# starreeze/drin

Measured on AMD Instinct MI355X. Metric: mention x candidate pairs scored/sec, higher is better.
Workload: dtype bf16x3; 1 GPU; wikimel-shaped scoring forward: 100-cand (+1 answer slot), D=768, R=2048, L=128, P=49, T=64 token-level entity text; parallelism=dp1 (mentions sharded, no collective)

## Files before the change

drin_amd/_lib.py:

```python
from __future__ import annotations

import ctypes as C
import os
from typing import Optional

_HERE = os.path.dirname(os.path.abspath(__file__))
LIB_PATH = os.environ.get("DRIN_LIB_PATH") or os.path.join(_HERE, "libdrin_hip.so")
MAX_LAYERS = 8
ABI_VERSION = 12

OK, E_SHAPE, E_NULL, E_ALIGN, E_WORKSPACE, E_HIP, E_UNSUPPORTED, E_INDEX = 0, -1, -2, -3, -4, -5, -6, -7
PREC_F32, PREC_BF16X3, PREC_BF16X3_ALL, PREC_BF16X3_IF16 = 0, 1, 3, 5
FEAT_F32, FEAT_BF16 = 0, 1
CACHE_F32, CACHE_MIXED_F16 = 0, 1
CACHE_FORMATS = {"f32": CACHE_F32, "mixed_f16": CACHE_MIXED_F16}
ACTIVATIONS = {"gelu": 1, "sigmoid": 2, "relu": 3, "tanh": 4, "silu": 5}

fp = C.POINTER(C.c_float)
ip = C.POINTER(C.c_int64)


class DrinConfigC(C.Structure):
    _fields_ = [
        ("batch", C.c_int32), ("num_candidates", C.c_int32), ("embed_dim", C.c_int32), ("image_dim", C.c_int32),
# ... 113 lines not shown
EXPORTS = {
    "drin_version": (C.c_int, []),
    "drin_last_error": (C.c_char_p, []),
    "drin_build_info": (C.c_char_p, []),
    "drin_default_config": (C.c_int, [C.POINTER(DrinConfigC)]),
    "drin_host_selftest": (C.c_int, []),
    "drin_workspace_bytes": (C.c_size_t, [C.POINTER(DrinConfigC), C.c_int]),
    "drin_edges_fwd": (C.c_int, [C.POINTER(DrinConfigC), C.POINTER(DrinBatchC), C.c_void_p, C.c_void_p, C.c_void_p]),
    "drin_pool_fwd": (C.c_int, [C.POINTER(DrinConfigC), C.POINTER(DrinBatchC), C.c_void_p, C.c_void_p, C.c_void_p, C.c_void_p]),
    "drin_linear_fwd": (C.c_int, [C.c_void_p, C.c_void_p, C.c_void_p, C.c_void_p, C.c_int64, C.c_int32, C.c_int32, C.c_int32, C.c_void_p]),
    "drin_linear_bwd": (C.c_int, [C.c_void_p, C.c_void_p, C.c_void_p, C.c_void_p, C.c_void_p, C.c_void_p, C.c_int64, C.c_int32,
                                  C.c_int32, C.c_int32, C.c_void_p, C.c_size_t, C.c_void_p]),
    "drin_forward": (C.c_int, [C.POINTER(DrinConfigC), C.POINTER(DrinBatchC), C.POINTER(DrinParamsC), C.c_void_p,
                               C.c_size_t, C.c_void_p, C.c_int, C.POINTER(DrinTraceC), C.c_void_p]),
    "drin_forward_staged": (C.c_int, [C.POINTER(DrinConfigC), C.POINTER(DrinBatchC), C.POINTER(DrinParamsC), C.c_void_p,
                                      C.c_size_t, C.c_void_p, C.c_int, C.POINTER(DrinTraceC), C.c_void_p, C.c_void_p]),
    "drin_backward": (C.c_int, [C.POINTER(DrinConfigC), C.POINTER(DrinBatchC), C.POINTER(DrinParamsC), C.c_void_p,
                                C.c_size_t, C.c_void_p, C.POINTER(DrinParamGradsC), C.c_void_p]),
    "drin_backward_staged": (C.c_int, [C.POINTER(DrinConfigC), C.POINTER(DrinBatchC), C.POINTER(DrinParamsC), C.c_void_p,
                                       C.c_size_t, C.c_void_p, C.POINTER(DrinParamGradsC), C.c_void_p, C.c_void_p]),
    "drin_backward_ex": (C.c_int, [C.POINTER(DrinConfigC), C.POINTER(DrinBatchC), C.POINTER(DrinParamsC), C.c_void_p,
                                   C.c_size_t, C.c_void_p, C.POINTER(DrinParamGradsC), C.POINTER(DrinInputGradsC), C.c_void_p,
                                   C.c_void_p]),
    "drin_input_grad_scratch_bytes": (C.c_size_t, [C.POINTER(DrinConfigC)]),
    "drin_pool_bwd": (C.c_int, [C.POINTER(DrinConfigC), C.c_void_p, C.c_void_p, C.c_void_p, C.c_void_p, C.c_void_p]),
    "drin_fused_supported": (C.c_int, [C.POINTER(DrinConfigC)]),
    "drin_indexed_supported": (C.c_int, [C.POINTER(DrinConfigC)]),
    "drin_prepared_bytes": (C.c_size_t, [C.POINTER(DrinConfigC)]),
    "drin_fused_workspace_bytes": (C.c_size_t, [C.POINTER(DrinConfigC)]),
    "drin_workgroups_per_mention": (C.c_int32, [C.POINTER(DrinConfigC), C.c_int32]),
    "drin_index_status": (C.c_int, [C.c_void_p, C.c_void_p]),
    "drin_image_contraction_passes": (C.c_int32, [C.POINTER(DrinConfigC), C.c_int32]),
    "drin_image_contraction_side_tiles": (C.c_int32, [C.POINTER(DrinConfigC), C.c_int32]),
    "drin_prepare": (C.c_int, [C.POINTER(DrinConfigC), C.POINTER(DrinParamsC), C.c_void_p, C.c_size_t, C.c_void_p]),
    "drin_forward_prepared": (C.c_int, [C.POINTER(DrinConfigC), C.POINTER(DrinBatchC), C.POINTER(DrinParamsC), C.c_void_p,
                                        C.c_void_p, C.c_size_t, C.c_void_p, C.c_void_p]),
    "drin_entity_cache_bytes": (C.c_size_t, [C.POINTER(DrinConfigC)]),
    "drin_entity_cache_build_workspace_bytes": (C.c_size_t, [C.POINTER(DrinConfigC)]),
    "drin_cached_workspace_bytes": (C.c_size_t, [C.POINTER(DrinConfigC)]),
    "drin_build_entity_cache": (C.c_int, [C.POINTER(DrinConfigC), C.POINTER(DrinBatchC), C.POINTER(DrinParamsC), C.c_void_p,
                                          C.c_void_p, C.c_size_t, C.c_void_p, C.c_size_t, C.c_void_p]),
    "drin_forward_cached": (C.c_int, [C.POINTER(DrinConfigC), C.POINTER(DrinBatchC), C.POINTER(DrinParamsC), C.c_void_p,
                                      C.c_void_p, C.c_void_p, C.c_size_t, C.c_void_p, C.c_void_p]),
    "drin_split_planes": (C.c_int, [C.c_void_p, C.c_void_p, C.c_void_p, C.c_int64, C.c_void_p]),
    "drin_linear_planes_fwd": (C.c_int, [C.c_void_p, C.c_void_p, C.c_void_p, C.c_void_p, C.c_void_p, C.c_void_p,
                                         C.c_int64, C.c_int32, C.c_int32, C.c_void_p]),
    "drin_gemm_probe": (C.c_int, [C.POINTER(DrinGemmProbeArgsC), C.c_void_p]),
    "drin_loss_workspace_bytes": (C.c_size_t, [C.c_int32]),
    "drin_triplet_topk": (C.c_int, [C.c_void_p, C.c_void_p, C.c_int32, C.c_int32, C.c_float, C.POINTER(C.c_int32), C.c_int32,
                                    C.c_void_p, C.c_void_p, C.c_void_p, C.c_void_p, C.c_size_t, C.c_void_p]),
    "drin_adam_step": (C.c_int, [C.c_void_p, C.c_void_p, C.c_void_p, C.c_void_p, C.c_int64, C.c_float, C.c_float, C.c_float,
                                 C.c_float, C.c_float, C.c_float, C.c_void_p]),
    "drin_melhi_workspace_bytes": (C.c_size_t, [C.POINTER(DrinMelhiConfigC), C.c_int]),
    "drin_melhi_forward": (C.c_int, [C.POINTER(DrinMelhiConfigC), C.POINTER(DrinMelhiBatchC), C.POINTER(DrinMelhiParamsC), C.c_void_p,
                                     C.c_void_p, C.c_void_p, C.c_size_t, C.c_void_p, C.c_void_p]),
    "drin_melhi_backward": (C.c_int, [C.POINTER(DrinMelhiConfigC), C.POINTER(DrinMelhiBatchC), C.POINTER(DrinMelhiParamsC),
                                      C.c_void_p, C.c_void_p, C.c_void_p, C.c_size_t, C.c_void_p, C.POINTER(DrinMelhiParamGradsC),
                                      C.c_void_p]),
    "drin_ghmfc_workspace_bytes": (C.c_size_t, [C.POINTER(DrinGhmfcConfigC)]),
    "drin_ghmfc_forward": (C.c_int, [C.POINTER(DrinGhmfcConfigC), C.POINTER(DrinGhmfcBatchC), C.POINTER(DrinGhmfcParamsC), C.c_void_p,
                                     C.c_size_t, C.c_void_p, C.c_void_p, C.c_void_p]),
    "drin_attention": (C.c_int, [C.c_void_p, C.c_int64, C.c_void_p, C.c_int64, C.c_void_p, C.c_int64, C.c_void_p, C.c_void_p, C.c_int64,
                                 C.c_int32, C.c_int32, C.c_int32, C.c_int32, C.c_int32, C.c_void_p]),
    "drin_attention_train_fwd": (C.c_int, [C.c_void_p, C.c_int64, C.c_void_p, C.c_int64, C.c_void_p, C.c_int64, C.c_void_p, C.c_void_p,
                                           C.c_int64, C.c_void_p, C.c_int32, C.c_int32, C.c_int32, C.c_int32, C.c_int32, C.c_void_p]),
    "drin_attention_bwd": (C.c_int, [C.c_void_p, C.c_int64, C.c_void_p, C.c_int64, C.c_void_p, C.c_int64, C.c_void_p, C.c_void_p,
                                     C.c_int64, C.c_void_p, C.c_void_p, C.c_int64, C.c_void_p, C.c_int64, C.c_void_p, C.c_int64,
                                     C.c_void_p, C.c_int64, C.c_void_p, C.c_int32, C.c_int32, C.c_int32, C.c_int32, C.c_int32,
                                     C.c_void_p]),
# ... 54 lines not shown
```

drin_amd/build.py:

```python
from __future__ import annotations

import os
import subprocess
import sys
from concurrent.futures import ThreadPoolExecutor

HERE = os.path.dirname(os.path.abspath(__file__))
CSRC = os.path.join(HERE, "csrc")
INCLUDE = os.path.join(os.path.dirname(HERE), "include")
LIB = os.path.join(HERE, "libdrin_hip.so")
ARCH = "gfx950"
SOURCES = ["api.hip", "stream_kernels.hip", "gemm_f32.hip", "gemm_bf16x3.hip", "gemm_x3_planes.hip", "gemm_tn_bf16x3.hip", "gcn_kernels.hip", "backward_kernels.hip", "fused_kernels.hip", "fused_forward.hip", "vector_kernels.hip", "loss_kernels.hip", "entity_cache.hip", "optim_kernels.hip", "input_grad_kernels.hip", "melhi_kernels.hip", "ghmfc_kernels.hip"]


def _hipcc() -> str:
    for c in (os.environ.get("HIPCC"), "/opt/rocm/bin/hipcc", "hipcc"):
        if c and (os.path.isabs(c) and os.path.exists(c) or not os.path.isabs(c)):
            return c
    raise RuntimeError("hipcc not found")


def _newest_header() -> float:
    hs = [os.path.join(CSRC, f) for f in os.listdir(CSRC) if f.endswith(".h")]
    hs += [os.path.join(INCLUDE, f) for f in os.listdir(INCLUDE) if f.endswith(".h")]
    return max(os.path.getmtime(h) for h in hs)


ASAN_LIB = os.path.join(HERE, "libdrin_hip_asan.so")
SAN_FLAGS = ["-fsanitize=address,undefined", "-fno-gpu-sanitize", "-fno-omit-frame-pointer", "-fno-sanitize-recover=undefined", "-g"]


def asan_runtime() -> str:
    out = subprocess.run([_hipcc(), "-print-file-name=libclang_rt.asan-x86_64.so"], capture_output=True, text=True).stdout.strip()
    if not os.path.isabs(out) or not os.path.exists(out):
        import glob
        hits = sorted(glob.glob("/opt/rocm/lib/llvm/lib/clang/*/lib/linux/libclang_rt.asan-x86_64.so"))
        if not hits:
            raise RuntimeError("clang's libclang_rt.asan-x86_64.so not found")
        out = hits[-1]
    return out


def build(force: bool = False, debug: bool = False, verbose: bool = True, asan_host: bool = False, variant: str = "") -> str:
    obj_dir = os.path.join(CSRC, "build_asan" if asan_host else ("build_" + variant if variant else "build"))
    os.makedirs(obj_dir, exist_ok=True)
# ... 49 lines not shown
```

drin_amd/csrc/fused.h:

```cpp
#pragma once
#include <hip/hip_runtime.h>
#include <stddef.h>
#include <stdint.h>
#include <string.h>

#include "../../include/drin_hip.h"
#include "layout.h"

namespace drin {

struct Prepared {
  size_t wcat1, bcat1, ecat, etmp, k_t, k_i, c_txt, c_img, cb_t, cb_i, total;
  size_t p_ctxt, p_cimg, p_wh2;
  size_t p_wmt, p_wmi, p_wcat1, p_ecat, p_wet, p_wei, p_wh1;
  size_t p_cimg_f16;
  size_t cimg_f16_scale;
  void build(const drin_config& c) {
    const size_t D = c.embed_dim, R = c.image_dim;
    size_t off = 0;
    auto take = [&off](size_t n) {
      const size_t o = off;
      off += (n + 63) & ~(size_t)63;
      return o;
    };
// ... 89 lines not shown
  const float* gamma;
  const float* beta;
  const float* e1m;
  const float* mt2;
  float* scores;
  int B, N, D4, chunks;
  int act_v;
  float ln_eps, cos_eps;
};

template <class Args>
Args shaped_args(const drin_config& c) {
  Args a;
  memset(&a, 0, sizeof(a));
  a.B = c.batch, a.N = c.num_candidates, a.D4 = c.embed_dim / 4;
  return a;
}
template <class Args>
void set_vertex_fields(Args& a, const drin_config& c) {
  a.ln_eps = c.layer_norm_eps, a.act_v = vertex_act(&c);
}
template <class Args>
void set_edge_fields(Args& a, const drin_config& c) {
  a.R4 = c.image_dim / 4;
  a.Km = c.mention_objects;
  a.dynamic = c.dynamic_edges != 0;
  a.act_e = edge_act(&c);
  for (int k = 0; k < 4; ++k) a.mask[k] = c.edge_enabled[k];
  a.cos_eps = c.cosine_eps, a.miei_eps = c.miei_eps, a.clip = c.clip_scale;
}

size_t entity_stream_lds_bytes(const StreamArgs& a);
int launch_entity_stream(const StreamArgs& a, hipStream_t st);
int launch_reduce_stream_partials(const float* part, float* s_text, float* s_img, float* sig, int B, int D, int R,
                                  int chunks, hipStream_t st);
int launch_mention_input1(const float* T, const float* T2, const float* sig, const float* b_et, const float* b_ei,
                          const float* v0, float* out, int B, int D, int N, hipStream_t st);
int launch_pair_layer1(const PairArgs& a, hipStream_t st);
int launch_mention_input2(const float* part, const float* mt1, float* out, int B, int D, int N, int chunks,
                          hipStream_t st);
int launch_pair_final(const FinalArgs& a, hipStream_t st);

struct GemmScratch {
  float* p = nullptr;
  size_t floats = 0;
};
int run_folded_head(const drin_config* cfg, const drin_batch* b, const drin_params* params, const float* prepared, const Prepared& P,
                    bool weight_planes, float* span_mean, float* mimg, float* vm0, float* hmfu, GemmScratch mention_sk, hipStream_t st);
int run_folded_mention_finish(const drin_config* cfg, const drin_params* params, const float* prepared, const Prepared& P,
                              bool weight_planes, float* vm1, float* hm2, GemmScratch mention_sk, hipStream_t st);
int run_folded_tail(const drin_config* cfg, const drin_params* params, const float* prepared, const Prepared& P, int chunks,
                    const float* s2_part, const float* vm1, float* agg2, float* mt2, const float* hm2, const float* e1m, float* h2,
                    const float* et1, const void* et1_hi, bool weight_planes, GemmScratch mention_sk, GemmScratch pair_sk,
                    float* scores, hipStream_t st);
}
```

drin_amd/csrc/fused_forward.hip:

```cpp
#include <string.h>

#include "fused.h"
#include "internal.h"
#include "layout.h"

namespace drin {

constexpr int kMixedMinCandidates = 64;

struct FusedLayout {
  size_t span_mean, mimg, vm0, hmfu, q, e0m, e1m, xt, s_part, s_text, s_img, sig, tm, tm2, agg1, vm1, hm2, h_text, h_image,
      et1, s2_part, agg2, mt2, p_xt, p_xi, p_et1, xi_scale, splitk, splitk_floats, pair_splitk, pair_splitk_floats, total;
  int chunks;
  void build(const drin_config& c) {
    const size_t B = c.batch, N = c.num_candidates, D = c.embed_dim, R = c.image_dim, M = B * N;
    chunks = (int)(B >= 2048 ? (N + 127) / 128 : B >= 1024 ? (N + 47) / 48 : (N + 15) / 16);
    size_t off = 0;
    auto take = [&off](size_t n) {
      const size_t o = off;
      off += (n + 63) & ~(size_t)63;
      return o;
    };
    span_mean = take(B * D);
    mimg = take(B * R);
// ... 63 lines not shown
#ifdef DRIN_SIDE_PROBE
static int g_probe_wgs = kSideWgs, g_probe_permille = kSidePermille;
extern "C" __attribute__((visibility("default"))) void drin_probe_side_plan(int wgs, int permille) { g_probe_wgs = wgs, g_probe_permille = permille; }
#endif
struct SidePlan {
  int64_t S = 0;
  int G = 0;
};
static SidePlan image_side_plan(const drin_config* c, bool indexed, bool capturing) {
  SidePlan plan;
  int wgs = kSideWgs, permille = kSidePermille;
#ifdef DRIN_SIDE_PROBE
  wgs = g_probe_wgs, permille = g_probe_permille;
#endif
  const bool split = c->precision == DRIN_PREC_BF16X3 || c->precision == DRIN_PREC_BF16X3_ALL || c->precision == DRIN_PREC_BF16X3_IF16;
  if (capturing || indexed || !split || if16_gate(c, indexed) || wgs <= 0 || permille <= 0) return plan;
  const int D = c->embed_dim, R = c->image_dim;
  if ((D % 32) || (R % 32) || c->batch <= 0) return plan;
  const int64_t M = (int64_t)c->batch * c->num_candidates;
  const int64_t nx = cdiv(D, 256), row_tiles = cdiv(M, 256), tiles = row_tiles * nx;
  if (tiles < 192 || tiles < kSideMinTiles || tiles > ((int64_t)1 << 28)) return plan;
  FusedLayout L;
  L.build(*c);
  const int64_t whole_rows = gemm_p4_whole_tiles(tiles, R, L.splitk_floats > 0, L.splitk_floats) / nx;
  int64_t S = (row_tiles * permille + 500) / 1000;
  S = S < whole_rows ? S : whole_rows;
  S = S < row_tiles - 1 ? S : row_tiles - 1;
  if (S <= 0) return plan;
  plan.S = S;
  plan.G = (int)(wgs < S * nx ? wgs : S * nx);
  return plan;
}

struct SideJoin {
  SideLane* lane = nullptr;
  hipStream_t st = nullptr;
  int join() {
    if (!lane) return DRIN_OK;
    const hipError_t e = hipStreamWaitEvent(st, lane->join, 0);
    lane = nullptr;
    return e == hipSuccess ? DRIN_OK : hip_fail(e, "hipStreamWaitEvent(side stream)");
  }
  ~SideJoin() { (void)join(); }
};

int fused_supported(const drin_config* c) {
  if (c->num_layers != 2) {
    set_error("fused path: built for num_layers == 2 (got %d); use drin_forward", c->num_layers);
    return DRIN_E_UNSUPPORTED;
  }
  if (c->vector_edges) {
    set_error("fused path: vector edge features (model.py:112-116) run on the layer-by-layer path; use drin_forward");
    return DRIN_E_UNSUPPORTED;
  }
  if (c->mention_object_inner > 1 || c->entity_object_inner > 1 || c->entity_image_inner > 1) {
    set_error("fused path: inner feature dims > 1 need the pooled path of drin_forward");
    return DRIN_E_UNSUPPORTED;
  }
  const bool tiny = c->embed_dim <= 256 && c->image_dim <= 256;
  const bool full = c->embed_dim <= 768 && c->image_dim <= 2048;
  if (!tiny && !full) {
    set_error("fused path: D=%d R=%d outside the built instantiations", c->embed_dim, c->image_dim);
    return DRIN_E_UNSUPPORTED;
  }
  return DRIN_OK;
}
// ... 138 lines not shown
                    const float* et1, const void* et1_hi, bool weight_planes, GemmScratch sk, GemmScratch pair_sk, float* scores,
                    hipStream_t st) {
  const int B = cfg->batch, N = cfg->num_candidates, D = cfg->embed_dim, prec = folded_precision(cfg);
  const int64_t M = (int64_t)B * N;
  const drin_layer_params& L2 = params->layer[1];
  DRIN_TRY(launch_mention_input2(s2_part, vm1, agg2, B, D, N, chunks, st));
  DRIN_TRY(launch_gemm_nt(agg2, D, L2.w_h, D, L2.b_h, mt2, D, B, D, D, false, prec, st, sk.p, sk.floats,
                          weight_planes ? pb + P.p_wh2 : nullptr));
  DRIN_TRY(launch_layernorm_gelu(mt2, L2.ln_weight, L2.ln_bias, mt2, nullptr, nullptr, B, D, cfg->layer_norm_eps, st, vertex_act(cfg)));
  if (et1_hi) {
    const __bf16* e1 = static_cast<const __bf16*>(et1_hi);
    const __bf16* w2 = reinterpret_cast<const __bf16*>(pb + P.p_wh2);
    DRIN_TRY(launch_gemm_x3_planes(e1, e1 + (size_t)M * D, D, w2, w2 + (size_t)D * D, D, nullptr, h2, D, M, D, D, st, pair_sk.p,
                                   pair_sk.floats));
  } else {
    DRIN_TRY(launch_gemm_nt(et1, D, L2.w_h, D, nullptr, h2, D, M, D, D, false, prec, st));
  }
  FinalArgs fa = shaped_args<FinalArgs>(*cfg);
  set_vertex_fields(fa, *cfg);
  fa.h2 = h2;
  fa.hm2 = hm2;
  fa.b_h2 = L2.b_h;
  fa.gamma = L2.ln_weight;
  fa.beta = L2.ln_bias;
  fa.e1m = e1m;
  fa.mt2 = mt2;
  fa.scores = scores;
  fa.chunks = chunks;
  fa.cos_eps = cfg->cosine_eps;
  return launch_pair_final(fa, st);
}

static int forward_prepared_on_stream(const drin_config* cfg, const drin_batch* b, const drin_params* params, const void* prepared,
                                      void* workspace, float* scores, hipStream_t st) {
  FusedLayout L;
  L.build(*cfg);
  Prepared P;
  P.build(*cfg);
  float* ws = (float*)workspace;
  const float* pb = (const float*)prepared;
  const int B = cfg->batch, N = cfg->num_candidates, D = cfg->embed_dim, R = cfg->image_dim;
  const int64_t M = (int64_t)B * N;
  if (B == 0) return DRIN_OK;
  const int prec = folded_precision(cfg);
  const bool dyn = cfg->dynamic_edges != 0;
  const bool tokens = cfg->entity_tokens > 0;
  const bool planes = (prec == DRIN_PREC_BF16X3 || prec == DRIN_PREC_BF16X3_ALL) && (D % 32 == 0) && (R % 32 == 0);
  const bool indexed = b->entity_index != nullptr;
  const bool xi_planes = planes && indexed;
  const bool if16 = if16_gate(cfg, indexed) && gemm_f16_planes_fits(ws + L.p_xi, R, pb + P.p_cimg_f16, R, ws + L.h_image, D, M, D, R);
  hipStreamCaptureStatus capture = hipStreamCaptureStatusNone;
  if (hipStreamIsCapturing(st, &capture) != hipSuccess) {
    (void)hipGetLastError();
    capture = hipStreamCaptureStatusActive;
  }
  SidePlan side = image_side_plan(cfg, indexed, capture != hipStreamCaptureStatusNone);
  if (!aligned16(b->entity_image) || !aligned16(ws + L.h_image) || !b->entity_image) side = SidePlan();
  if (b->entity_text_cls) {
    set_error("drin_forward_prepared: entity_text_cls (text pooled ahead of time) is a form of the training entry points");
    return DRIN_E_UNSUPPORTED;
  }
  if (indexed && cfg->num_entities <= 0) {
    set_error("drin_forward_prepared: entity_index given but cfg.num_entities = %d", cfg->num_entities);
    return DRIN_E_SHAPE;
  }
  if (indexed && !planes) {
    set_error("drin_forward_prepared: entity_index needs the split-bf16 precision (the stream kernel gathers the "
// ... 55 lines not shown
  sa.index_status = b->index_status;
  sa.miet = b->miet_similarity;
  sa.mtei = b->mtei_similarity;
  sa.span_mean = ws + L.span_mean;
  sa.mobj = b->mention_object;
  sa.mscore = b->mention_object_score;
  sa.fu = hmfu + D;
  sa.ldfu = 2 * D;
  sa.q = ws + L.q;
  sa.ldq = D + R;
  sa.k_t = pb + P.k_t;
  sa.k_i = pb + P.k_i;
  sa.xt_out = planes ? nullptr : ws + L.xt;
  if (planes) {
    sa.xt_hi = xt_hi;
    sa.xt_lo = xt_exact ? nullptr : xt_hi + MD;
    if (xi_planes) {
      sa.xi_hi = xi_hi;
      sa.xi_lo = bf16_feat ? nullptr : xi_hi + MR;
    }
  }
  sa.xi_scale = if16 ? ws + L.xi_scale : nullptr;
  sa.xi_f16 = if16 ? static_cast<void*>(xi_hi) : nullptr;
  sa.e0m = ws + L.e0m;
  sa.e1m = ws + L.e1m;
  sa.s_part = ws + L.s_part;
  sa.T = cfg->entity_tokens;
  sa.Ke = cfg->entity_objects;
  sa.chunks = L.chunks;
  sa.bf16_features = bf16_feat ? 1 : 0;
  sa.s_text = ws + L.s_text;
  sa.s_img = ws + L.s_img;
  sa.sig = ws + L.sig;
  DRIN_TRY(launch_entity_stream(sa, st));
  if (L.chunks > 1)
    DRIN_TRY(launch_reduce_stream_partials(ws + L.s_part, ws + L.s_text, ws + L.s_img, ws + L.sig, B, D, R, L.chunks, st));
  DRIN_TRY(launch_gemm_nt_pair({ws + L.s_text, params->w_entity_text, nullptr, ws + L.tm, D, D, D, 2 * (int64_t)B, D, D, wp(P.p_wet)},
                               {ws + L.s_img, params->w_entity_image, nullptr, ws + L.tm2, R, R, D, 2 * (int64_t)B, D, R,
                                wp(P.p_wei)},
                               prec, st, msk.p, msk.floats));
  DRIN_TRY(launch_mention_input1(ws + L.tm, ws + L.tm2, ws + L.sig, params->b_entity_text, params->b_entity_image, vm0, ws + L.agg1, B, D, N, st));
  float* vm1 = ws + L.vm1;
  DRIN_TRY(launch_gemm_nt(ws + L.agg1, D, L1.w_h, D, L1.b_h, vm1, D, 2 * (int64_t)B, D, D, false, prec, st, msk.p, msk.floats, wp(P.p_wh1)));
  DRIN_TRY(run_folded_mention_finish(cfg, params, pb, P, planes, vm1, ws + L.hm2, msk, st));
  if (planes) {
    const __bf16* ct = reinterpret_cast<const __bf16*>(pb + P.p_ctxt);
    const __bf16* ci = reinterpret_cast<const __bf16*>(pb + P.p_cimg);
    DRIN_TRY(launch_gemm_x3_planes(xt_hi, xt_exact ? nullptr : xt_hi + MD, D, ct, ct + (size_t)D * D, D, nullptr, ws + L.h_text, D, M, D,
                                   D, st, psk.p, psk.floats));
    if (if16)
      DRIN_TRY(launch_gemm_f16_planes(xi_hi, R, pb + P.p_cimg_f16, R, ws + L.xi_scale, pb + P.cimg_f16_scale, ws + L.h_image, D, M, D, R,
                                      st, psk.p, psk.floats));
    else if (xi_planes)
      DRIN_TRY(launch_gemm_x3_planes(xi_hi, bf16_feat ? nullptr : xi_hi + MR, R, ci, ci + (size_t)D * R, R, nullptr, ws + L.h_image, D, M,
                                     D, R, st, psk.p, psk.floats));
    else if (side.S > 0) {
      DRIN_TRY(side_join.join());
      DRIN_TRY(image_rows_product(st, RowTiles{side.S, -1, 0}));
    } else if (bf16_feat)
      DRIN_TRY(launch_gemm_x3_planes(b->entity_image, nullptr, R, ci, ci + (size_t)D * R, R, nullptr, ws + L.h_image, D, M, D, R, st, psk.p,
                                     psk.floats));
    else
      DRIN_TRY(launch_gemm_nt_bf16x3(b->entity_image, R, pb + P.c_img, R, nullptr, ws + L.h_image, D, M, D, R, st, ci, ci + (size_t)D * R,
                                     false, psk.p, psk.floats));
  } else {
    const float* x_t = tokens ? ws + L.xt : b->entity_text;
    DRIN_TRY(launch_gemm_nt(x_t, D, pb + P.c_txt, D, nullptr, ws + L.h_text, D, M, D, D, false, prec, st));
    DRIN_TRY(launch_gemm_nt(b->entity_image, R, pb + P.c_img, R, nullptr, ws + L.h_image, D, M, D, R, false, prec, st));
  }
// ... 8 lines not shown
  pa.gamma = L1.ln_weight;
  pa.beta = L1.ln_bias;
  pa.e0m = ws + L.e0m;
  pa.e1m = ws + L.e1m;
  pa.et1 = planes ? nullptr : ws + L.et1;
  if (planes) {
    pa.et1_hi = e1_hi;
    pa.et1_lo = e1_hi + MD;
  }
  pa.s2_part = ws + L.s2_part;
  pa.chunks = L.chunks;
  DRIN_TRY(launch_pair_layer1(pa, st));
  return run_folded_tail(cfg, params, pb, P, L.chunks, ws + L.s2_part, vm1, ws + L.agg2, ws + L.mt2, ws + L.hm2, ws + L.e1m, ws + L.h_text,
                         planes ? nullptr : ws + L.et1, planes ? e1_hi : nullptr, planes, msk, psk, scores, st);
}

}

extern "C" {

int32_t drin_workgroups_per_mention(const drin_config* cfg, int32_t cached) {
  if (validate_config(cfg) != DRIN_OK || fused_supported(cfg) != DRIN_OK) return 0;
  if (cached) return cached_chunks_per_mention(*cfg);
  FusedLayout L;
  L.build(*cfg);
  return L.chunks;
}

int32_t drin_image_contraction_side_tiles(const drin_config* cfg, int32_t indexed) {
  if (validate_config(cfg) != DRIN_OK || fused_supported(cfg) != DRIN_OK) return 0;
  return (int32_t)image_side_plan(cfg, indexed != 0, false).S;
}

int32_t drin_image_contraction_passes(const drin_config* cfg, int32_t indexed) {
  if (validate_config(cfg) != DRIN_OK || fused_supported(cfg) != DRIN_OK) return 0;
  if (cfg->precision == DRIN_PREC_F32) return 0;
  if (if16_gate(cfg, indexed != 0)) return 1;
  return cfg->feature_dtype == DRIN_FEAT_BF16 ? 2 : 3;
}

int drin_index_status(int32_t* index_status, void* stream) {
  if (!index_status) {
    set_error("drin_index_status: NULL argument");
    return DRIN_E_NULL;
  }
  DRIN_BIND_DEVICE(stream, index_status, "drin_index_status");
  int32_t w[4] = {0, 0, 0, 0};
  hipError_t e = hipMemcpyAsync(w, index_status, sizeof(w), hipMemcpyDeviceToHost, (hipStream_t)stream);
  if (e == hipSuccess) e = hipStreamSynchronize((hipStream_t)stream);
  if (e != hipSuccess) return hip_fail(e, "drin_index_status");
  if (w[0] == 0) return DRIN_OK;
  e = hipMemsetAsync(index_status, 0, sizeof(w), (hipStream_t)stream);
  if (e != hipSuccess) return hip_fail(e, "drin_index_status(reset)");
  const long long value = (long long)(((uint64_t)(uint32_t)w[3] << 32) | (uint32_t)w[2]);
  set_error("entity_index out of range: candidate row %lld at pair %d (b * N + n) is outside the entity tables - the row was clamped "
            "and a WRONG entity scored; drin/data.py:87-93 raises IndexError here", value, (int)w[1]);
  return DRIN_E_INDEX;
}

size_t drin_fused_workspace_bytes(const drin_config* cfg) {
  if (validate_config(cfg) != DRIN_OK || fused_supported(cfg) != DRIN_OK) return 0;
  FusedLayout L;
  L.build(*cfg);
  return L.total * sizeof(float);
}

int drin_forward_prepared(const drin_config* cfg, const drin_batch* b, const drin_params* params, const void* prepared,
                          void* workspace, size_t workspace_bytes, float* scores, void* stream) {
  DRIN_BIND_DEVICE(stream, workspace, "drin_forward_prepared");
  RoctxRange range("drin_forward_prepared");
  DRIN_TRY(validate_config(cfg));
  DRIN_TRY(fused_supported(cfg));
  if (!b || !params || !prepared || !workspace || !scores) {
    set_error("drin_forward_prepared: NULL argument");
    return DRIN_E_NULL;
  }
  FusedLayout L;
  L.build(*cfg);
  if (workspace_bytes < L.total * sizeof(float) || !aligned16(workspace)) {
    set_error("drin_forward_prepared: workspace has %zu bytes (needs %zu) or is not 16-byte aligned", workspace_bytes,
              L.total * sizeof(float));
    return DRIN_E_WORKSPACE;
  }
  return forward_prepared_on_stream(cfg, b, params, prepared, workspace, scores, (hipStream_t)stream);
}

}
```

include/drin_hip.h:

```cpp
#ifndef DRIN_HIP_H_
#define DRIN_HIP_H_

#include <stddef.h>
#include <stdint.h>

#ifdef __cplusplus
extern "C" {
#endif

#define DRIN_ABI_VERSION 12
#define DRIN_API __attribute__((visibility("default")))

typedef enum {
  DRIN_OK = 0,
  DRIN_E_SHAPE = -1,
  DRIN_E_NULL = -2,
  DRIN_E_ALIGN = -3,
  DRIN_E_WORKSPACE = -4,
  DRIN_E_HIP = -5,
  DRIN_E_UNSUPPORTED = -6,
  DRIN_E_INDEX = -7
} drin_status;

typedef enum {
// ... 141 lines not shown
                 void* workspace, size_t workspace_bytes, float* scores, int keep_for_backward,
                 const drin_trace* trace, void* params_ready_event, void* stream);

DRIN_API int drin_backward(const drin_config* cfg, const drin_batch* batch, const drin_params* params,
                  void* workspace, size_t workspace_bytes, const float* grad_scores,
                  const drin_param_grads* grads, void* stream);

DRIN_API int drin_backward_staged(const drin_config* cfg, const drin_batch* batch, const drin_params* params,
                  void* workspace, size_t workspace_bytes, const float* grad_scores,
                  const drin_param_grads* grads, void* layers_ready_event, void* stream);

DRIN_API int drin_backward_ex(const drin_config* cfg, const drin_batch* batch, const drin_params* params,
                              void* workspace, size_t workspace_bytes, const float* grad_scores,
                              const drin_param_grads* grads, const drin_input_grads* input_grads,
                              void* layers_ready_event, void* stream);
DRIN_API size_t drin_input_grad_scratch_bytes(const drin_config* cfg);

DRIN_API int drin_pool_bwd(const drin_config* cfg, const int64_t* entity_text_mask, const float* grad_pooled,
                           const float* grad_cls, void* grad_entity_text, void* stream);

DRIN_API int drin_fused_supported(const drin_config* cfg);
DRIN_API size_t drin_prepared_bytes(const drin_config* cfg);
DRIN_API size_t drin_fused_workspace_bytes(const drin_config* cfg);
DRIN_API int drin_prepare(const drin_config* cfg, const drin_params* params, void* prepared, size_t prepared_bytes,
                          void* stream);
DRIN_API int drin_forward_prepared(const drin_config* cfg, const drin_batch* batch, const drin_params* params,
                                   const void* prepared, void* workspace, size_t workspace_bytes, float* scores,
                                   void* stream);
DRIN_API int32_t drin_workgroups_per_mention(const drin_config* cfg, int32_t cached);

DRIN_API int32_t drin_image_contraction_passes(const drin_config* cfg, int32_t indexed);

DRIN_API int32_t drin_image_contraction_side_tiles(const drin_config* cfg, int32_t indexed);

DRIN_API int drin_index_status(int32_t* index_status, void* stream);

DRIN_API size_t drin_entity_cache_bytes(const drin_config* cfg);
DRIN_API size_t drin_entity_cache_build_workspace_bytes(const drin_config* cfg);
DRIN_API size_t drin_cached_workspace_bytes(const drin_config* cfg);
DRIN_API int drin_build_entity_cache(const drin_config* cfg, const drin_batch* tables, const drin_params* params,
                                     const void* prepared, void* cache, size_t cache_bytes, void* workspace,
                                     size_t workspace_bytes, void* stream);
DRIN_API int drin_forward_cached(const drin_config* cfg, const drin_batch* batch, const drin_params* params,
                                 const void* prepared, const void* cache, void* workspace, size_t workspace_bytes,
                                 float* scores, void* stream);

DRIN_API int drin_split_planes(const float* x, void* hi, void* lo, int64_t n, void* stream);
DRIN_API int drin_linear_planes_fwd(const void* x_hi, const void* x_lo, const void* w_hi, const void* w_lo,
                                    const float* bias, float* y, int64_t rows, int32_t n_out, int32_t k,
                                    void* stream);

enum drin_gemm_probe_op {
  DRIN_PROBE_GEMM_NT = 1,
  DRIN_PROBE_GEMM_NT_BF16X3 = 2,
  DRIN_PROBE_GEMM_NT_BF16X3_P4 = 3,
  DRIN_PROBE_GEMM_X3_PLANES = 4,
  DRIN_PROBE_GEMM_F16_PLANES = 5,
  DRIN_PROBE_TO_F16_SCALED = 6
};
enum drin_gemm_family {
  DRIN_GEMM_FAMILY_NONE = 0,
  DRIN_GEMM_FAMILY_BF16X3 = 1,
  DRIN_GEMM_FAMILY_BF16X3_P4 = 2,
  DRIN_GEMM_FAMILY_PLANES = 3,
  DRIN_GEMM_FAMILY_PLANES_P4 = 4,
  DRIN_GEMM_FAMILY_F32 = 5,
// ... 184 lines not shown
```

Measured before the change: 28.06 million pairs/s.

## Add workgroup-per-mention walk kernel for the entity stream pass

Adds a new kernel that assigns one 256-thread workgroup per mention. The four waves split the token rows of each candidate, and the next candidate's rows are prefetched while the current one is reduced. When the config fits (fp32 features, D=768, R=2048, one entity object row, more than 16 candidates, a single chunk), it replaces the pair-per-wave entity stream kernel and the partial-reduction launch. The intent is better memory-level parallelism across token rows and fewer launches, at the cost of only B workgroups in the grid and heavy LDS use that may limit occupancy. A probe entry point is added to force either path.

```diff
diff --git a/drin_amd/_lib.py b/drin_amd/_lib.py
--- a/drin_amd/_lib.py
+++ b/drin_amd/_lib.py
@@ -169,9 +169,12 @@
     "drin_index_status": (C.c_int, [C.c_void_p, C.c_void_p]),
     "drin_image_contraction_passes": (C.c_int32, [C.POINTER(DrinConfigC), C.c_int32]),
     "drin_image_contraction_side_tiles": (C.c_int32, [C.POINTER(DrinConfigC), C.c_int32]),
+    "drin_stream_walk": (C.c_int32, [C.POINTER(DrinConfigC), C.c_int32]),
     "drin_prepare": (C.c_int, [C.POINTER(DrinConfigC), C.POINTER(DrinParamsC), C.c_void_p, C.c_size_t, C.c_void_p]),
     "drin_forward_prepared": (C.c_int, [C.POINTER(DrinConfigC), C.POINTER(DrinBatchC), C.POINTER(DrinParamsC), C.c_void_p,
                                         C.c_void_p, C.c_size_t, C.c_void_p, C.c_void_p]),
+    "drin_forward_prepared_probe": (C.c_int, [C.POINTER(DrinConfigC), C.POINTER(DrinBatchC), C.POINTER(DrinParamsC), C.c_void_p,
+                                              C.c_void_p, C.c_size_t, C.c_void_p, C.c_int32, C.c_void_p]),
     "drin_entity_cache_bytes": (C.c_size_t, [C.POINTER(DrinConfigC)]),
     "drin_entity_cache_build_workspace_bytes": (C.c_size_t, [C.POINTER(DrinConfigC)]),
     "drin_cached_workspace_bytes": (C.c_size_t, [C.POINTER(DrinConfigC)]),
diff --git a/drin_amd/build.py b/drin_amd/build.py
--- a/drin_amd/build.py
+++ b/drin_amd/build.py
@@ -10,7 +10,7 @@
 INCLUDE = os.path.join(os.path.dirname(HERE), "include")
 LIB = os.path.join(HERE, "libdrin_hip.so")
 ARCH = "gfx950"
-SOURCES = ["api.hip", "stream_kernels.hip", "gemm_f32.hip", "gemm_bf16x3.hip", "gemm_x3_planes.hip", "gemm_tn_bf16x3.hip", "gcn_kernels.hip", "backward_kernels.hip", "fused_kernels.hip", "fused_forward.hip", "vector_kernels.hip", "loss_kernels.hip", "entity_cache.hip", "optim_kernels.hip", "input_grad_kernels.hip", "melhi_kernels.hip", "ghmfc_kernels.hip"]
+SOURCES = ["api.hip", "stream_kernels.hip", "gemm_f32.hip", "gemm_bf16x3.hip", "gemm_x3_planes.hip", "gemm_tn_bf16x3.hip", "gcn_kernels.hip", "backward_kernels.hip", "fused_kernels.hip", "stream_walk.hip", "fused_forward.hip", "vector_kernels.hip", "loss_kernels.hip", "entity_cache.hip", "optim_kernels.hip", "input_grad_kernels.hip", "melhi_kernels.hip", "ghmfc_kernels.hip"]
 
 
 def _hipcc() -> str:
diff --git a/drin_amd/csrc/fused.h b/drin_amd/csrc/fused.h
--- a/drin_amd/csrc/fused.h
+++ b/drin_amd/csrc/fused.h
@@ -145,6 +145,9 @@
 
 size_t entity_stream_lds_bytes(const StreamArgs& a);
 int launch_entity_stream(const StreamArgs& a, hipStream_t st);
+bool mention_walk_built(const StreamArgs& a);
+size_t mention_walk_lds_bytes(const StreamArgs& a);
+int launch_mention_walk(const StreamArgs& a, hipStream_t st);
 int launch_reduce_stream_partials(const float* part, float* s_text, float* s_img, float* sig, int B, int D, int R,
                                   int chunks, hipStream_t st);
 int launch_mention_input1(const float* T, const float* T2, const float* sig, const float* b_et, const float* b_ei,
diff --git a/drin_amd/csrc/fused_forward.hip b/drin_amd/csrc/fused_forward.hip
--- a/drin_amd/csrc/fused_forward.hip
+++ b/drin_amd/csrc/fused_forward.hip
@@ -119,6 +119,17 @@
   return plan;
 }
 
+static bool stream_walk_built(const drin_config* c, bool indexed) {
+  return !indexed && c->feature_dtype == DRIN_FEAT_F32 && c->entity_tokens > 0 && c->embed_dim == 768 && c->image_dim == 2048 &&
+         c->entity_objects == 1 && c->mention_objects <= 11 && c->precision != DRIN_PREC_BF16X3_IF16;
+}
+static int stream_walk_route(const drin_config* c, bool indexed) {
+  if (!stream_walk_built(c, indexed) || c->num_candidates <= 16) return 0;
+  FusedLayout L;
+  L.build(*c);
+  return L.chunks == 1 ? 1 : 0;
+}
+
 struct SideJoin {
   SideLane* lane = nullptr;
   hipStream_t st = nullptr;
@@ -323,7 +334,7 @@
 }
 
 static int forward_prepared_on_stream(const drin_config* cfg, const drin_batch* b, const drin_params* params, const void* prepared,
-                                      void* workspace, float* scores, hipStream_t st) {
+                                      void* workspace, float* scores, hipStream_t st, int forced_walk = -1) {
   FusedLayout L;
   L.build(*cfg);
   Prepared P;
@@ -445,9 +456,15 @@
   sa.s_text = ws + L.s_text;
   sa.s_img = ws + L.s_img;
   sa.sig = ws + L.sig;
-  DRIN_TRY(launch_entity_stream(sa, st));
-  if (L.chunks > 1)
-    DRIN_TRY(launch_reduce_stream_partials(ws + L.s_part, ws + L.s_text, ws + L.s_img, ws + L.sig, B, D, R, L.chunks, st));
+  const int walk = forced_walk < 0 ? stream_walk_route(cfg, indexed) : forced_walk;
+  if (walk == 1) {
+    sa.chunks = 1;
+    DRIN_TRY(launch_mention_walk(sa, st));
+  } else {
+    DRIN_TRY(launch_entity_stream(sa, st));
+    if (L.chunks > 1)
+      DRIN_TRY(launch_reduce_stream_partials(ws + L.s_part, ws + L.s_text, ws + L.s_img, ws + L.sig, B, D, R, L.chunks, st));
+  }
   DRIN_TRY(launch_gemm_nt_pair({ws + L.s_text, params->w_entity_text, nullptr, ws + L.tm, D, D, D, 2 * (int64_t)B, D, D, wp(P.p_wet)},
                                {ws + L.s_img, params->w_entity_image, nullptr, ws + L.tm2, R, R, D, 2 * (int64_t)B, D, R,
                                 wp(P.p_wei)},
@@ -522,6 +539,11 @@
   return (int32_t)image_side_plan(cfg, indexed != 0, false).S;
 }
 
+int32_t drin_stream_walk(const drin_config* cfg, int32_t indexed) {
+  if (validate_config(cfg) != DRIN_OK || fused_supported(cfg) != DRIN_OK) return 0;
+  return stream_walk_route(cfg, indexed != 0);
+}
+
 int32_t drin_image_contraction_passes(const drin_config* cfg, int32_t indexed) {
   if (validate_config(cfg) != DRIN_OK || fused_supported(cfg) != DRIN_OK) return 0;
   if (cfg->precision == DRIN_PREC_F32) return 0;
@@ -555,24 +577,50 @@
   return L.total * sizeof(float);
 }
 
+static int forward_prepared_checked(const char* who, const drin_config* cfg, const drin_batch* b, const drin_params* params,
+                                    const void* prepared, void* workspace, size_t workspace_bytes, float* scores, int forced_walk,
+                                    void* stream) {
+  DRIN_TRY(validate_config(cfg));
+  DRIN_TRY(fused_supported(cfg));
+  if (!b || !params || !prepared || !workspace || !scores) {
+    set_error("%s: NULL argument", who);
+    return DRIN_E_NULL;
+  }
+  if (forced_walk > 1 || forced_walk < -1) {
+    set_error("%s: stream_walk %d (0: a pair per wave, 1: a pair per workgroup)", who, forced_walk);
+    return DRIN_E_SHAPE;
+  }
+  if (forced_walk == 1 && !stream_walk_built(cfg, b->entity_index != nullptr)) {
+    set_error("%s: the workgroup walk of the entity stream pass is built for fp32-stored gathered rows with token features at D = 768, "
+              "R = 2048, one entity object row and no fp16 image hand-over", who);
+    return DRIN_E_UNSUPPORTED;
+  }
+  FusedLayout L;
+  L.build(*cfg);
+  if (workspace_bytes < L.total * sizeof(float) || !aligned16(workspace)) {
+    set_error("%s: workspace has %zu bytes (needs %zu) or is not 16-byte aligned", who, workspace_bytes, L.total * sizeof(float));
+    return DRIN_E_WORKSPACE;
+  }
+  return forward_prepared_on_stream(cfg, b, params, prepared, workspace, scores, (hipStream_t)stream, forced_walk);
+}
+
 int drin_forward_prepared(const drin_config* cfg, const drin_batch* b, const drin_params* params, const void* prepared,
                           void* workspace, size_t workspace_bytes, float* scores, void* stream) {
   DRIN_BIND_DEVICE(stream, workspace, "drin_forward_prepared");
   RoctxRange range("drin_forward_prepared");
-  DRIN_TRY(validate_config(cfg));
-  DRIN_TRY(fused_supported(cfg));
-  if (!b || !params || !prepared || !workspace || !scores) {
-    set_error("drin_forward_prepared: NULL argument");
-    return DRIN_E_NULL;
-  }
-  FusedLayout L;
-  L.build(*cfg);
-  if (workspace_bytes < L.total * sizeof(float) || !aligned16(workspace)) {
-    set_error("drin_forward_prepared: workspace has %zu bytes (needs %zu) or is not 16-byte aligned", workspace_bytes,
-              L.total * sizeof(float));
-    return DRIN_E_WORKSPACE;
-  }
-  return forward_prepared_on_stream(cfg, b, params, prepared, workspace, scores, (hipStream_t)stream);
-}
-
-}
+  return forward_prepared_checked("drin_forward_prepared", cfg, b, params, prepared, workspace, workspace_bytes, scores, -1, stream);
+}
+
+int drin_forward_prepared_probe(const drin_config* cfg, const drin_batch* b, const drin_params* params, const void* prepared,
+                                void* workspace, size_t workspace_bytes, float* scores, int32_t stream_walk, void* stream) {
+  DRIN_BIND_DEVICE(stream, workspace, "drin_forward_prepared_probe");
+  RoctxRange range("drin_forward_prepared_probe");
+  if (stream_walk != 0 && stream_walk != 1) {
+    set_error("drin_forward_prepared_probe: stream_walk %d (0: a pair per wave, 1: a pair per workgroup)", (int)stream_walk);
+    return DRIN_E_SHAPE;
+  }
+  return forward_prepared_checked("drin_forward_prepared_probe", cfg, b, params, prepared, workspace, workspace_bytes, scores,
+                                  (int)stream_walk, stream);
+}
+
+}
diff --git a/drin_amd/csrc/stream_walk.hip b/drin_amd/csrc/stream_walk.hip
--- /dev/null
+++ b/drin_amd/csrc/stream_walk.hip
@@ -0,0 +1,291 @@
+#include "device_utils.h"
+#include "fused.h"
+#include "internal.h"
+#include "row_ops.h"
+
+namespace drin {
+
+namespace {
+constexpr int kD = 768, kR = 2048, kD4 = kD / 4;
+constexpr int kSlots = 16, kSlotObj = 5;
+
+__device__ __forceinline__ void lds_barrier() {
+  asm volatile("s_waitcnt lgkmcnt(0)" ::: "memory");
+  __builtin_amdgcn_s_barrier();
+  asm volatile("" ::: "memory");
+}
+__device__ __forceinline__ float sum_waves(const float* tab, int slot) {
+  return ((tab[slot] + tab[kSlots + slot]) + tab[2 * kSlots + slot]) + tab[3 * kSlots + slot];
+}
+__device__ __forceinline__ float4 zero4() { return make_float4(0.f, 0.f, 0.f, 0.f); }
+}
+
+__global__ void __launch_bounds__(256, 2) k_mention_walk(const StreamArgs a) {
+  extern __shared__ __attribute__((aligned(16))) float lds[];
+  const float* const f_text = static_cast<const float*>(a.entity_text);
+  const float* const f_image = static_cast<const float*>(a.entity_image);
+  const float* const f_object = static_cast<const float*>(a.entity_object);
+  const float* const f_mobj = static_cast<const float*>(a.mobj);
+  constexpr int D4 = kD4, R4 = kR / 4, D = kD, R = kR;
+  float* l_mobj = lds;
+  float* l_q = l_mobj + a.Km * R;
+  float* l_mt = l_q + 2 * R;
+  float* l_part = l_mt + 3 * D;
+  float* l_tab = l_part + 4 * D;
+  float* l_tab2 = l_tab + 4 * kSlots;
+  float* l_small = l_tab2 + 8;
+  const int tid = threadIdx.x, wave = __builtin_amdgcn_readfirstlane(tid >> 6), lane = tid & 63;
+  const int64_t b = blockIdx.y;
+  const int N = a.N, T = a.T, Km = a.Km;
+  const bool dyn = a.dynamic != 0;
+  const bool txt = wave < 3;
+  const int rc = (128 * wave + lane) * 4;
+
+  for (int i = tid; i < Km * R4; i += 256) st4(l_mobj + i * 4, ld4(f_mobj + (b * Km) * R + i * 4));
+  for (int i = tid; i < D4; i += 256) st4(l_mt + i * 4, ld4(a.span_mean + b * D + i * 4));
+  if (dyn) {
+    for (int i = tid; i < 2 * R4; i += 256) {
+      const int which = i / R4, c4 = i - which * R4;
+      st4(l_q + i * 4, ld4(a.q + ((int64_t)which * a.B + b) * a.ldq + D + c4 * 4));
+    }
+    for (int i = tid; i < 2 * D4; i += 256) {
+      const int which = i / D4, c4 = i - which * D4;
+      st4(l_mt + D + i * 4, ld4(a.q + ((int64_t)which * a.B + b) * a.ldq + c4 * 4));
+    }
+  }
+  if (tid < Km) l_small[Km + tid] = a.mscore[b * Km + tid];
+  __syncthreads();
+  for (int i = wave; i < Km; i += 4) {
+    float s = 0.f;
+    for (int c4 = lane; c4 < R4; c4 += 64) {
+      const float4 v = ld4(l_mobj + i * R + c4 * 4);
+      s += dot4(v, v);
+    }
+    s = wave_sum(s);
+    if (lane == 0) l_small[i] = fmaxf(sqrtf(s), a.cos_eps);
+  }
+  float m_t_norm;
+  {
+    const Row<3> m_t = load_row<3>(l_mt, lane, D4);
+    m_t_norm = fmaxf(sqrtf(wave_sum(dot_rows<3>(m_t, m_t))), a.cos_eps);
+  }
+  float kap_tt = 0.f, kap_ti = 0.f, kap_it = 0.f, kap_ii = 0.f;
+  if (dyn) {
+    const Row<3> fu_t = load_row<3>(a.fu + b * a.ldfu, lane, D4);
+    const Row<3> fu_i = load_row<3>(a.fu + ((int64_t)a.B + b) * a.ldfu, lane, D4);
+    const Row<3> k_t = load_row<3>(a.k_t, lane, D4), k_i = load_row<3>(a.k_i, lane, D4);
+    kap_tt = wave_sum(dot_rows<3>(fu_t, k_t));
+    kap_ti = wave_sum(dot_rows<3>(fu_t, k_i));
+    kap_it = wave_sum(dot_rows<3>(fu_i, k_t));
+    kap_ii = wave_sum(dot_rows<3>(fu_i, k_i));
+  }
+  __syncthreads();
+
+  float4 S_tt = zero4(), S_it = zero4();
+  float4 S_ti[2] = {zero4(), zero4()}, S_ii[2] = {zero4(), zero4()};
+  float sg_tt = 0.f, sg_ti = 0.f, sg_it = 0.f, sg_ii = 0.f;
+  const float inv_d = 1.0f / (float)D;
+  const int64_t p0 = b * N, M = (int64_t)a.B * N;
+
+  auto mask_words = [&](int64_t p) {
+    int c = 0;
+    for (int t = lane; t < T; t += 64) c += (int)a.entity_mask[p * T + t];
+    return c;
+  };
+  auto slice_stop = [&](int c) {
+    const int cnt = (int)wave_sum((float)c);
+    int stop = cnt - 1;
+    if (stop < 0) stop += T;
+    return stop < 0 ? 0 : (stop > T ? T : stop);
+  };
+  float4 tok[8][3];
+  auto request_rows = [&](int64_t p, int stop, int k0) {
+    const float* base = f_text + p * (int64_t)T * D + lane * 4;
+#pragma unroll
+    for (int u = 0; u < 8; ++u) {
+      const int t = 1 + wave + 4 * (k0 + u);
+      if (t < stop) {
+#pragma unroll
+        for (int j = 0; j < 3; ++j) tok[u][j] = ld4_stream(base + (int64_t)t * D + 256 * j);
+      } else {
+#pragma unroll
+        for (int j = 0; j < 3; ++j) tok[u][j] = zero4();
+      }
+    }
+  };
+  float4 cls, eo[2], xin[2];
+  float es, mtei, miet;
+  int words_next = 0;
+  auto request_pair = [&](int n, int stop) {
+    const int64_t p = p0 + n;
+    request_rows(p, stop, 0);
+    cls = txt ? ld4_stream(f_text + p * (int64_t)T * D + tid * 4) : zero4();
+#pragma unroll
+    for (int j = 0; j < 2; ++j) {
+      eo[j] = ld4_stream(f_object + p * R + rc + 256 * j);
+      xin[j] = ld4_stream(f_image + p * R + rc + 256 * j);
+    }
+    es = a.entity_object_score[p];
+    mtei = a.mtei[p];
+    miet = a.miet[p];
+    words_next = n + 1 < N ? mask_words(p + 1) : 0;
+  };
+
+  int stop = slice_stop(mask_words(p0));
+  request_pair(0, stop);
+  for (int n = 0; n < N; ++n) {
+    const int64_t p = p0 + n;
+    float4 acc[3] = {zero4(), zero4(), zero4()};
+#pragma unroll
+    for (int u = 0; u < 8; ++u)
+#pragma unroll
+      for (int j = 0; j < 3; ++j) acc[j] = acc[j] + tok[u][j];
+    for (int k0 = 8; 1 + wave + 4 * k0 < stop; k0 += 8) {
+      request_rows(p, stop, k0);
+#pragma unroll
+      for (int u = 0; u < 8; ++u)
+#pragma unroll
+        for (int j = 0; j < 3; ++j) acc[j] = acc[j] + tok[u][j];
+    }
+#pragma unroll
+    for (int j = 0; j < 3; ++j) st4(l_part + wave * D + (lane + 64 * j) * 4, acc[j]);
+    {
+      const float xy = wave_sum(txt ? dot4(cls, ld4(l_mt + tid * 4)) : 0.f);
+      const float yy = wave_sum(dot4(cls, cls));
+      const float oo = wave_sum(dot4(eo[0], eo[0]) + dot4(eo[1], eo[1]));
+      float* tab = l_tab + wave * kSlots;
+      if (lane == 0) tab[0] = xy, tab[1] = yy, tab[2] = oo;
+      if (dyn) {
+        const float ti = wave_sum(dot4(xin[0], ld4(l_q + rc)) + dot4(xin[1], ld4(l_q + rc + 256)));
+        const float ii = wave_sum(dot4(xin[0], ld4(l_q + R + rc)) + dot4(xin[1], ld4(l_q + R + rc + 256)));
+        if (lane == 0) tab[3] = ti, tab[4] = ii;
+      }
+      for (int i = 0; i < Km; ++i) {
+        const float om = wave_sum(dot4(eo[0], ld4(l_mobj + i * R + rc)) + dot4(eo[1], ld4(l_mobj + i * R + rc + 256)));
+        if (lane == 0) tab[kSlotObj + i] = om;
+      }
+    }
+    const float4 xi0 = xin[0], xi1 = xin[1];
+    const float es_n = es, mtei_n = mtei, miet_n = miet;
+    const int stop_n = stop;
+    if (n + 1 < N) {
+      stop = slice_stop(words_next);
+      request_pair(n + 1, stop);
+    }
+    lds_barrier();
+    float4 xt = zero4();
+    if (txt) {
+      const float4 s = ((ld4(l_part + tid * 4) + ld4(l_part + D + tid * 4)) + ld4(l_part + 2 * D + tid * 4)) + ld4(l_part + 3 * D + tid * 4);
+      const float den = stop_n > 1 ? (float)(stop_n - 1) : 0.0f;
+      xt = make_float4(s.x / den, s.y / den, s.z / den, s.w / den);
+    }
+    if (dyn) {
+      const float tt = wave_sum(txt ? dot4(xt, ld4(l_mt + D + tid * 4)) : 0.f);
+      const float it = wave_sum(txt ? dot4(xt, ld4(l_mt + 2 * D + tid * 4)) : 0.f);
+      if (lane == 0) l_tab2[2 * wave] = tt, l_tab2[2 * wave + 1] = it;
+    }
+    const float xy = sum_waves(l_tab, 0), yy = sum_waves(l_tab, 1);
+    const float ny = fmaxf(sqrtf(sum_waves(l_tab, 2)), a.cos_eps);
+    float d_ti = 0.f, d_ii = 0.f;
+    if (dyn) d_ti = sum_waves(l_tab, 3), d_ii = sum_waves(l_tab, 4);
+    float sim = 0.f, wsum = 0.f;
+    for (int i = 0; i < Km; ++i) {
+      const float w = l_small[Km + i] * es_n;
+      sim += sum_waves(l_tab, kSlotObj + i) / (l_small[i] * ny) * w;
+      wsum += w;
+    }
+    lds_barrier();
+    if (txt) {
+      if (a.xt_out) st4(a.xt_out + p * D + tid * 4, xt);
+      if (a.xt_hi) {
+        bf16x4_t h, l;
+        split_bf16x4(xt, h, l);
+        __builtin_nontemporal_store(h, reinterpret_cast<bf16x4_t*>(reinterpret_cast<__bf16*>(a.xt_hi) + p * D + tid * 4));
+        if (a.xt_lo) __builtin_nontemporal_store(l, reinterpret_cast<bf16x4_t*>(reinterpret_cast<__bf16*>(a.xt_lo) + p * D + tid * 4));
+      }
+    }
+    const float tt = xy / (m_t_norm * fmaxf(sqrtf(yy), a.cos_eps));
+    const float ii = sim / (wsum + a.miei_eps);
+    const float e_tt = tt * a.mask[0];
+    const float e_ti = (mtei_n / a.clip) * a.mask[1];
+    const float e_it = (miet_n / a.clip) * a.mask[2];
+    const float e_ii = ii * a.mask[3];
+    if (tid == 0) {
+      float n_tt = e_tt, n_ti = e_ti, n_it = e_it, n_ii = e_ii;
+      if (dyn) {
+        const float d_tt = ((l_tab2[0] + l_tab2[2]) + l_tab2[4]) + l_tab2[6];
+        const float d_it = ((l_tab2[1] + l_tab2[3]) + l_tab2[5]) + l_tab2[7];
+        n_tt = edge_act_apply(a.act_e, (d_tt + kap_tt) * inv_d + e_tt);
+        n_ti = edge_act_apply(a.act_e, (d_ti + kap_ti) * inv_d + e_ti);
+        n_it = edge_act_apply(a.act_e, (d_it + kap_it) * inv_d + e_it);
+        n_ii = edge_act_apply(a.act_e, (d_ii + kap_ii) * inv_d + e_ii);
+      }
+      a.e0m[p] = e_tt;
+      a.e0m[M + p] = e_ti;
+      a.e0m[2 * M + p] = e_it;
+      a.e0m[3 * M + p] = e_ii;
+      a.e1m[p] = n_tt * a.mask[0];
+      a.e1m[M + p] = n_ti * a.mask[1];
+      a.e1m[2 * M + p] = n_it * a.mask[2];
+      a.e1m[3 * M + p] = n_ii * a.mask[3];
+    }
+    S_tt = fma4(e_tt, xt, S_tt);
+    S_it = fma4(e_it, xt, S_it);
+    S_ti[0] = fma4(e_ti, xi0, S_ti[0]);
+    S_ti[1] = fma4(e_ti, xi1, S_ti[1]);
+    S_ii[0] = fma4(e_ii, xi0, S_ii[0]);
+    S_ii[1] = fma4(e_ii, xi1, S_ii[1]);
+    sg_tt += e_tt;
+    sg_ti += e_ti;
+    sg_it += e_it;
+    sg_ii += e_ii;
+  }
+
+  if (txt) {
+    st4(a.s_text + b * D + tid * 4, S_tt);
+    st4(a.s_text + ((int64_t)a.B + b) * D + tid * 4, S_it);
+  }
+#pragma unroll
+  for (int j = 0; j < 2; ++j) {
+    st4(a.s_img + b * R + rc + 256 * j, S_ti[j]);
+    st4(a.s_img + ((int64_t)a.B + b) * R + rc + 256 * j, S_ii[j]);
+  }
+  if (tid == 0) {
+    a.sig[b] = sg_tt;
+    a.sig[(int64_t)a.B + b] = sg_ti;
+    a.sig[2 * (int64_t)a.B + b] = sg_it;
+    a.sig[3 * (int64_t)a.B + b] = sg_ii;
+  }
+}
+
+size_t mention_walk_lds_bytes(const StreamArgs& a) {
+  return sizeof(float) * ((size_t)a.Km * kR + 2 * kR + 3 * kD + 4 * kD + 4 * kSlots + 8 + 2 * (size_t)a.Km);
+}
+
+bool mention_walk_built(const StreamArgs& a) {
+  return a.D4 == kD4 && a.R4 == kR / 4 && a.T > 0 && !a.bf16_features && a.entity_index == nullptr && a.xi_hi == nullptr &&
+         a.xi_scale == nullptr && a.xi_f16 == nullptr && a.chunks == 1 && a.Ke == 1 && a.Km >= 0 && a.Km <= kSlots - kSlotObj;
+}
+
+int launch_mention_walk(const StreamArgs& a, hipStream_t st) {
+  if (a.B <= 0) return DRIN_OK;
+  if (!mention_walk_built(a)) {
+    set_error("entity stream pass: the workgroup walk is built for fp32 gathered rows with token features at D = 768, R = 2048, one "
+              "entity object row, at most %d mention objects and one workgroup per mention", kSlots - kSlotObj);
+    return DRIN_E_UNSUPPORTED;
+  }
+  if (a.B > 65535) {
+    set_error("entity_stream: batch %d exceeds the grid limit; split the batch", a.B);
+    return DRIN_E_SHAPE;
+  }
+  const size_t lds = mention_walk_lds_bytes(a);
+  static DynLdsOptIn opt_in;
+  if (lds > 48 * 1024)
+    DRIN_TRY(ensure_dynamic_lds(opt_in, reinterpret_cast<const void*>(k_mention_walk), (int)lds, "hipFuncSetAttribute(mention_walk)"));
+  KernelTimer timer(DRIN_KC_STREAM, st);
+  hipLaunchKernelGGL(k_mention_walk, dim3(1u, (unsigned)a.B), dim3(256), lds, st, a);
+  DRIN_CHECK_LAUNCH("k_mention_walk");
+  return DRIN_OK;
+}
+
+}
diff --git a/include/drin_hip.h b/include/drin_hip.h
--- a/include/drin_hip.h
+++ b/include/drin_hip.h
@@ -197,6 +197,12 @@
 DRIN_API int32_t drin_image_contraction_passes(const drin_config* cfg, int32_t indexed);
 
 DRIN_API int32_t drin_image_contraction_side_tiles(const drin_config* cfg, int32_t indexed);
+
+DRIN_API int32_t drin_stream_walk(const drin_config* cfg, int32_t indexed);
+
+DRIN_API int drin_forward_prepared_probe(const drin_config* cfg, const drin_batch* batch, const drin_params* params,
+                                         const void* prepared, void* workspace, size_t workspace_bytes, float* scores,
+                                         int32_t stream_walk, void* stream);
 
 DRIN_API int drin_index_status(int32_t* index_status, void* stream);
 
```

Result: slower. 26.63 million pairs/s (-5.1%).
